# thethomasboyer/PhenDiff

Measured on AMD Instinct MI355X. Metric: img2img images/sec (50-step DDIM invert+denoise, 256x256), higher is better.
Workload: dtype bf16; 1 GPU; configs[2]: 256x256 pipeline_conditional_ddim invert->class-swap->denoise, 50+50 DDIM steps, super_small UNet (random init, seed 0), 3k_steps_clipping_rescaling, 32 images/GPU/step sharded over 1 GPU(s), no collectives; batch_per_gpu=32, global_batch=32, inference_steps=50, image_size=256, hipgraph=True, concurrent_trajectories=1

## Files before the change

### include/phendiff_hip.h

```cpp
#ifndef PHENDIFF_HIP_H_
#define PHENDIFF_HIP_H_

#include <stddef.h>
#include <stdint.h>

#ifdef __cplusplus
extern "C" {
#endif

#define PD_ABI_VERSION 8

typedef enum { PD_OK = 0, PD_ERR_ARG = -1, PD_ERR_SHAPE = -2, PD_ERR_LAUNCH = -3, PD_ERR_UNSUPPORTED = -4 } pd_status;
typedef enum { PD_F32 = 0, PD_BF16 = 1, PD_F16 = 2 } pd_dtype;
typedef enum { PD_PRED_EPSILON = 0, PD_PRED_SAMPLE = 1, PD_PRED_V = 2 } pd_pred_type;

int pd_abi_version(void);
const char* pd_last_error(void);

typedef struct {
  int rows;
  int c0;
  int tdim;
  int proj_dim;
  int flip_sin_to_cos;
// ... 44 lines not shown
  int Hout, Wout;
  int C0, C1;
  int Cout;
  int Cout_pad;
  int ksize;
  int stride;
  int pad;
  int upsample;
  int silu;
  int out_mode;
  int heads;
  const void* x0; const void* x1;
  const float* scale; const float* shift;
  const void* w_packed;
  const float* bias;
  const float* temb; int temb_stride;
  const void* residual;
  void* y;
  float* stats_out;
  const void* tail_x0; const void* tail_x1; int tail_C0, tail_C1;
  int im2col3;
  int phase;
  int phase_in;
} pd_conv_args;
int pd_conv(const pd_conv_args* a, void* stream);
int pd_conv_stat_tiles(int Hout, int Wout, int ksize, int stride);

typedef struct {
  int B, HW, groups; float eps;
  int C0, T0; const float* stats0;
  int C1, T1; const float* stats1;
  const float* gamma; const float* beta;
  float* scale; float* shift;
  float* mean; float* rstd;
  const float* temb; int temb_stride;
} pd_gn_finalize_args;
int pd_gn_finalize(const pd_gn_finalize_args* a, void* stream);

typedef struct {
  int dtype;
  int B, heads, N;
  const void* q; const void* k; const void* v;
  void* out;
  float* lse;
  const float* kmax2;
} pd_attn_args;
// ... 663 lines not shown
```

### phendiff_amd/csrc/conv_igemm.hip

```cpp
#include <type_traits>
#include <utility>
#include <stdio.h>
#include <stdlib.h>
#include "pd_common.h"
#include "pd_stage.h"
#include "pd_conv.h"

namespace pd {

constexpr int CONV_AR8 = 6;
constexpr int CONV_PRO_DEFAULT = 1;
constexpr int CONV_PRO_WPS = 3;
constexpr int CONV_PRO_START = 8;
template <int... I, typename F> __device__ __forceinline__ void pd_static_for_impl(std::integer_sequence<int, I...>, F&& f) { (f(std::integral_constant<int, I>{}), ...); }
template <int N, typename F> __device__ __forceinline__ void pd_static_for(F&& f) { pd_static_for_impl(std::make_integer_sequence<int, N>{}, f); }
constexpr int PRO_OPS = 37;
constexpr int pro_op_cost(int k) {
  if (k >= 36) return 100;
  const int stg = (k % 18) >> 1;
  return (stg == 3 || stg == 4 || stg == 6 || stg == 7) ? 87 : (stg == 0 ? 60 : (stg == 8 ? 106 : 58));
}
constexpr int pro_ops_done(int S, int NS, int PS0, int NIT) {
  if (S < PS0) return 0;
  if (S >= NS - 1) return NIT * PRO_OPS;
  long long tot = 0;
  for (int k = 0; k < PRO_OPS; ++k) tot += pro_op_cost(k);
  tot *= NIT;
  const long long target = (long long)(S - PS0 + 1) * tot / (NS - PS0);
  int done = 0;
  long long dc = 0;
  while (done < NIT * PRO_OPS && dc + pro_op_cost(done % PRO_OPS) <= target) { dc += pro_op_cost(done % PRO_OPS); ++done; }
  return done;
}
__device__ __forceinline__ unsigned pd_lin_block() { return blockIdx.x + gridDim.x * (blockIdx.y + gridDim.y * blockIdx.z); }
template <typename T, int KS, int STRIDE, int TH, int TW, bool DB, bool TAIL, int NCO = 1, bool PLAIN = false, int PRO = 0, bool STACK = false>
__global__ __launch_bounds__(256, NCO == 2 ? 2 : (PRO ? CONV_PRO_WPS : (((KS == 1 || (KS == 3 && STRIDE == 1 && TH * TW == 256)) && sizeof(T) == 2) ? 3 : 2))) void conv_kernel(const ConvP p) {
  static_assert(PRO == 0 || (!PLAIN && DB && KS == 3 && STRIDE == 1 && sizeof(T) == 2), "compile-time prologue: 16-bit 3x3 stride-1 double-buffered launches");
  static_assert(!TAIL || (DB && KS == 3 && STRIDE == 1), "fused shortcut tail: 3x3 stride-1 double-buffered variant only");
  static_assert(NCO == 1 || (NCO == 2 && DB && KS == 3 && STRIDE == 1), "two output tiles per workgroup: 3x3 stride-1 double-buffered variant only");
  static_assert(!STACK || (KS == 3 && STRIDE == 1 && TW == 8 && TH == 16 && NCO == 1 && !PLAIN && PRO == 0), "stacked 8 x 8 images: the 16 x 8 tile");
  constexpr int SG = STACK ? TH / 8 : 1;
  using E = Elem<T>;
  using Frag = typename E::Frag;
  using SR = typename Stage<T>::R;
  constexpr int TP = TH * TW;
  constexpr int NF = TP / 64;
  constexpr int RPF = 32 / TW;
  constexpr int IN_TH = STACK ? SG * 10 : (TH - 1) * STRIDE + KS;
  constexpr int IN_TW = (TW - 1) * STRIDE + KS;
  constexpr int NPIX = IN_TH * IN_TW;
  constexpr bool M16 = PLAIN && sizeof(T) == 2 && (KS == 3 || KS == 2) && STRIDE == 1 && DB && TW >= 16;
  constexpr int CHB = 32 * E::BYTES;
  constexpr int PITCH = DB ? 2 * CHB + (M16 ? 32 : 16) : CHB + 16;
  constexpr int NIT = (NPIX * 4 + 255) / 256;
  constexpr int TAPS = KS * KS;
  constexpr int KSTEPS = TAPS * 2;
  constexpr int LDS_TILE = DB ? CHB : 0;
  static_assert(RPF >= 1 && TW * RPF == 32, "TW must divide 32");

  extern __shared__ __attribute__((aligned(16))) unsigned char lds[];

  int co_t = blockIdx.y, n = blockIdx.z * SG, bx = blockIdx.x;
  if (!STACK && p.co_major) {
    const int gx = gridDim.x, gxz = gridDim.x * gridDim.z;
    const int idx = xcd_chunk_index((int)pd_lin_block(), gxz * (int)gridDim.y);
    co_t = idx / gxz;
    const int rem = idx - co_t * gxz;
    n = rem / gx; bx = rem - n * gx;
  }
  int tx, ty;
  if (p.tiles_x_shift >= 0) { tx = bx & (p.tiles_x - 1); ty = bx >> p.tiles_x_shift; }
  else { ty = bx / p.tiles_x; tx = bx - ty * p.tiles_x; }
  const int y0 = ty * TH, x0 = tx * TW;

  const int tid = threadIdx.x;
  const int lane = tid & 63;
  const int wave = __builtin_amdgcn_readfirstlane(tid >> 6);
  const int wp = wave >> 1, wc = wave & 1;
  const int r = lane & 31, h = lane >> 5;
  const int ct32 = co_t * (2 * NCO) + wc;
  const bool wave_active = (ct32 * 32) < p.Cout_pad;

  const __amdgpu_buffer_rsrc_t rs0 = __builtin_amdgcn_make_buffer_rsrc((void*)p.x0, 0, p.bytes0, 0x00020000);
  const __amdgpu_buffer_rsrc_t rs1 = __builtin_amdgcn_make_buffer_rsrc((void*)(p.x1 ? p.x1 : p.x0), 0, p.bytes1, 0x00020000);

  const __amdgpu_buffer_rsrc_t rt0 = __builtin_amdgcn_make_buffer_rsrc((void*)(TAIL ? p.t0 : p.x0), 0, TAIL ? p.tbytes0 : p.bytes0, 0x00020000);
  const __amdgpu_buffer_rsrc_t rt1 = __builtin_amdgcn_make_buffer_rsrc((void*)((TAIL && p.t1) ? p.t1 : p.x0), 0, (TAIL && p.t1) ? p.tbytes1 : p.bytes0, 0x00020000);

  const int sub = tid & 3;
  auto stage_pix = [&](int i) { return (tid + 256 * i) >> 2; };
  const int Hc = p.upsample ? p.Hin * 2 : p.Hin;
  const int Wc = p.upsample ? p.Win * 2 : p.Win;
  int spix[NIT];
  constexpr int TAIL_CENTRE = 1 << 30;
  const int ups = p.upsample ? 1 : 0;
  const int ph_mask = p.upsample >= 2 ? 1 : 0, ph_want = p.upsample == 3 ? 1 : 0;
  const int istep = p.in_step, Ws = p.Win * istep;
  const int iy_base = y0 * STRIDE - p.pad, ix_base = x0 * STRIDE - p.pad_x, n_base = n * p.Hin * istep + p.in_oy;
#pragma unroll
  for (int i = 0; i < NIT; ++i) {
    const int pix = stage_pix(i);
    const int u = pix / IN_TW, vv = pix - u * IN_TW;
    const int sj = STACK ? u / 10 : 0, su = u - sj * 10;
    const int iy = STACK ? su - 1 : iy_base + u, ix = ix_base + vv;
    const bool ok = (pix < NPIX) & ((unsigned)iy < (unsigned)Hc) & ((unsigned)ix < (unsigned)Wc) & (!STACK || n + sj < p.B)
                    & (((iy & ph_mask) == (ph_want & ph_mask)) & ((ix & ph_mask) == (ph_want & ph_mask)));
    int v = STACK ? ((n + sj) * 8 + iy) * 8 + ix : (n_base + (iy >> ups) * istep) * Ws + (ix >> ups) * istep + p.in_ox;
    if (TAIL) v |= (((unsigned)((STACK ? su : u) - KS / 2) < (unsigned)(STACK ? 8 : TH)) & ((unsigned)(vv - KS / 2) < (unsigned)TW)) ? TAIL_CENTRE : 0;
    spix[i] = ok ? v : -1;
  }
  const bool affine = PRO || (!PLAIN && p.scale != nullptr);
  const bool do_silu = PRO || (!PLAIN && p.silu != 0);
  const int cin = p.C0 + p.C1;

  SR stage[NIT];
  float sc[8], sh[8];
  bool stage_plain = false;
  auto issue_loads = [&](int chunk) {
    int src, cch;
    if (!TAIL || chunk < p.n_main) { cch = chunk * 32; src = cch < p.C0 ? 0 : 1; if (src == 1) cch -= p.C0; }
    else { cch = (chunk - p.n_main) * 32; src = cch < p.Ct0 ? 2 : 3; if (src == 3) cch -= p.Ct0; }
// ... 79 lines not shown
  };

  auto frag_row = [&](int fi, int q) { return fi * RPF + q; };
  const int li = lane & 15, lg = lane >> 4;
  constexpr int TJ_STEP = (TW >= 32 ? 16 : IN_TW) * PITCH;
  int rbase[NF];
#pragma unroll
  for (int f = 0; f < NF; ++f) {
    const int fi = wp * NF + f;
    if constexpr (M16) {
      rbase[f] = f == 0 ? ((wp * NF * RPF) * IN_TW + li) * PITCH + lg * 8 * E::BYTES : 0;
    } else {
      const int py = frag_row(fi, r / TW), px = r % TW;
      const int ly = STACK ? py + 2 * (py >> 3) : py * STRIDE;
      rbase[f] = (ly * IN_TW + px * STRIDE) * PITCH + h * 8 * E::BYTES;
    }
  }

  f32x16 acc[NCO][NF];
  f32x4 acq[NCO][NF][4];
  const int main_ksteps = (TAIL ? p.n_main : p.nchunks) * KSTEPS;
  const int all_ksteps = main_ksteps + (TAIL ? p.n_tail * 2 : 0);
  const unsigned wfrag = 512u * E::BYTES;
  const __amdgpu_buffer_rsrc_t rw = __builtin_amdgcn_make_buffer_rsrc((void*)p.w, 0, (unsigned)(p.Cout_pad / 32) * (unsigned)all_ksteps * wfrag, 0x00020000);
  const unsigned wlane = (unsigned)lane * 8u * E::BYTES;
  const unsigned wtile = (unsigned)ct32 * (unsigned)all_ksteps * wfrag;
  const unsigned wstep = 2u * (unsigned)all_ksteps * wfrag;
  auto load_w = [&](int c, int kstep) { return E::load_buf(rw, wlane, wtile + (unsigned)c * wstep + (unsigned)kstep * wfrag); };

  constexpr int AR = (KS == 3 && TW == 8 && STRIDE == 1 && sizeof(T) == 2 && TP <= 128) ? CONV_AR8 : ((KSTEPS % 3 == 0) ? 3 : 2);
  static_assert(KSTEPS % AR == 0, "the ring index is static");
  constexpr int AD = AR - 1;
  Frag aring[AR][NCO];
  static_assert(!M16 || NF % 2 == 0, "M16 walks a fragment pair per half-step");
  Frag aq[2][NCO][2];
  const unsigned wlane16 = (unsigned)(((lg >> 1) * 64 + (lg & 1) * 32 + li) * 16);
  auto load_w16 = [&](int c, int tap_index, int ti) {
    return E::load_buf(rw, wlane16 + (unsigned)ti * 256u, wtile + (unsigned)c * wstep + (unsigned)(2 * tap_index) * wfrag);
  };

  auto mma_chunk = [&](int chunk, const unsigned char* buf, unsigned char* nbuf, auto have_next_c, auto active_c) {
    constexpr int NEXT = (int)decltype(have_next_c)::value;
    constexpr bool HAVE_NEXT = NEXT != 0, NEXT_PLAIN = NEXT == 2;
    constexpr bool ACTIVE = decltype(active_c)::value;
    const int g0 = chunk * KSTEPS;
    Frag bc[NF];
    int piece = 0;
// ... 323 lines not shown
#pragma unroll
        for (int i = 0; i < 4; ++i)
          if (co + i < p.Cout) ((float*)p.y)[(((size_t)n * p.Cout + co + i) * p.Hout + oy) * p.Wout + ox] = acc[0][f][4 * g + i];
      }
    }
    return;
  }
  constexpr int EP_PITCH = 64 * E::BYTES + 16;
  constexpr int EPC = 16 / E::BYTES;
  constexpr int PPP = 64 / EPC;
  constexpr int PXI = 256 / PPP;
  constexpr int NEP = TP / PXI;
  static_assert(PXI % TW == 0 || TW % PXI == 0, "epilogue piece map");
  const int piece = tid % PPP, prow = tid / PPP;
  const int py0 = prow / TW, px0 = prow % TW;
  const int os = p.out_step, HF = p.Hout * os, WF = p.Wout * os;
  const unsigned out_bytes = (unsigned)p.B * HF * WF * p.Cout * E::BYTES;
  const __amdgpu_buffer_rsrc_t ry = __builtin_amdgcn_make_buffer_rsrc((void*)p.y, 0, p.out_mode == PD_OUT_NHWC ? out_bytes : 0u, 0x00020000);
  const __amdgpu_buffer_rsrc_t rres = __builtin_amdgcn_make_buffer_rsrc((void*)(p.residual ? p.residual : p.y), 0, p.residual ? out_bytes : 0u, 0x00020000);
  const unsigned px_bytes = (unsigned)p.Cout * E::BYTES * os, row_bytes = (unsigned)WF * p.Cout * E::BYTES * os;
  auto piece_off = [&](int it, int co) -> unsigned {
    const int dpy = (it * PXI) / TW, dpx = (it * PXI) % TW;
    const int oy = y0 + py0 + dpy, ox = x0 + px0 + dpx;
    const unsigned off = (unsigned)((n * HF + (y0 + py0) * os + p.out_oy) * WF + (x0 + px0) * os + p.out_ox) * (unsigned)(p.Cout * E::BYTES)
                         + (unsigned)co * E::BYTES + (unsigned)dpy * row_bytes + (unsigned)dpx * px_bytes;
    if constexpr (STACK) return (n + ((py0 + dpy) >> 3) < p.B && co < p.Cout) ? off : OOB_OFF;
    return (oy < p.Hout && ox < p.Wout && co < p.Cout) ? off : OOB_OFF;
  };
  if (!DB) __syncthreads();
#pragma unroll
  for (int cth = 0; cth < NCO; ++cth) {
  const int co_tile = co_t * NCO + cth;
  const int co = co_tile * 64 + piece * EPC;
  u32x4 rr[NEP];
  if (p.out_mode == PD_OUT_NHWC) {
#pragma unroll
    for (int it = 0; it < NEP; ++it) rr[it] = __builtin_amdgcn_raw_buffer_load_b128(rres, piece_off(it, co), 0, 0);
  }
  if (cth > 0) __syncthreads();
  if (wave_active) {
    if constexpr (M16) {
#pragma unroll
      for (int f = 0; f < NF; ++f)
#pragma unroll
        for (int q = 0; q < 4; ++q) {
          const int plin = (wp * NF + f) * 32 + (q & 1) * 16 + li;
          const f32x4 v = acq[cth][f][q];
// ... 67 lines not shown
    }
  }
  if (p.stats) {
    float* red = (float*)(lds + TP * EP_PITCH);
#pragma unroll
    for (int sg = 0; sg < SG; ++sg) {
      if (sg > 0) __syncthreads();
#pragma unroll
      for (int q = 0; q < 2 * EPC / 4; ++q) {
        f32x4 v4;
#pragma unroll
        for (int j = 0; j < 4; ++j) { const int e = q * 4 + j; v4[j] = e < EPC ? ssum[sg][e] : ssq[sg][e - EPC]; }
        *(f32x4*)(red + tid * (2 * EPC) + q * 4) = v4;
      }
      __syncthreads();
      if (tid < 128) {
        const int c = tid >> 1, which = tid & 1;
        const int pc = c / EPC, j = c % EPC;
        const int cog = co_tile * 64 + c;
        float tot = 0.f;
#pragma unroll 8
        for (int pr = 0; pr < PXI; ++pr) tot += red[(pr * PPP + pc) * (2 * EPC) + which * EPC + j];
        if (cog < p.Cout && n + sg < p.B) {
          const int tile = p.stat_tile_base + ty * p.tiles_x + tx;
          p.stats[(((size_t)(n + sg) * p.stat_tiles + tile) * p.Cout + cog) * 2 + which] = tot;
        }
      }
    }
  }
  }
}

template <typename T, int KS, int STRIDE, int TH, int TW, bool TAIL = false, int NCO = 1, bool PLAIN = false, int PRO = 0, bool STACK = false>
static int launch_conv(const ConvP& p, hipStream_t st) {
  constexpr int IN_TH = STACK ? (TH / 8) * 10 : (TH - 1) * STRIDE + KS, IN_TW = (TW - 1) * STRIDE + KS;
  constexpr int PITCH = 32 * Elem<T>::BYTES + 16;
  constexpr int LDS_TILE = ((IN_TH * IN_TW * PITCH + 15) / 16) * 16;
  constexpr bool DB = 2 * LDS_TILE <= 100 * 1024 && STRIDE != 2;
  constexpr bool M16 = PLAIN && sizeof(T) == 2 && (KS == 3 || KS == 2) && STRIDE == 1 && TW >= 16;
  constexpr int LDS_DB = ((IN_TH * IN_TW * (2 * 32 * Elem<T>::BYTES + (M16 ? 32 : 16)) + 15) / 16) * 16;
  constexpr int EPI_BYTES = TH * TW * (64 * Elem<T>::BYTES + 16) + 256 * 64;
  constexpr int LDS_MAIN = (DB ? LDS_DB : LDS_TILE) + (PRO ? 16 : 0);
  constexpr int LDS_BYTES = LDS_MAIN > EPI_BYTES ? LDS_MAIN : EPI_BYTES;
  static_assert(LDS_BYTES <= 160 * 1024, "tile too large");
  static_assert(NCO == 1 || DB, "NCO = 2 is a double-buffered variant");
  auto kern = conv_kernel<T, KS, STRIDE, TH, TW, DB, TAIL, NCO, PLAIN, PRO, STACK>;
  if (LDS_BYTES > 64 * 1024) {
    static LdsAttr attr;
    if (!ensure_lds(attr, kern, LDS_BYTES)) { set_error("pd_conv: cannot reserve %d bytes of LDS", LDS_BYTES); return PD_ERR_LAUNCH; }
  }
  ConvP q = p;
  q.tiles_x = (p.Wout + TW - 1) / TW;
  q.tiles_y = STACK ? 1 : (p.Hout + TH - 1) / TH;
  q.tiles_x_shift = -1;
  for (int sft = 0; sft < 16; ++sft) if ((1 << sft) == q.tiles_x) q.tiles_x_shift = sft;
  q.n_co_tiles = (p.Cout_pad + 63) / 64;
  if (q.stat_tiles == 0) q.stat_tiles = q.tiles_x * q.tiles_y;
  else { q.stat_tiles *= q.tiles_x * q.tiles_y; q.stat_tile_base *= q.tiles_x * q.tiles_y; }
  {
    const long long es = (long long)sizeof(T), cin = (long long)p.C0 + p.C1;
    const long long wbytes = (long long)p.Cout_pad * cin * KS * KS * es, abytes = (long long)p.B * p.Hin * p.Win * cin * es;
    const long long blocks = (long long)q.tiles_x * q.tiles_y * (q.n_co_tiles / NCO) * p.B;
    const int env = diag_env("PD_CONV_XCD", 0);
    q.co_major = !STACK && blocks >= 64 && blocks < (1ll << 30) && !p.im2col3 && (env == 1 || (env == 2 && wbytes > abytes));
  }
  hipLaunchKernelGGL(kern, dim3(q.tiles_x * q.tiles_y, q.n_co_tiles / NCO, STACK ? (p.B + TH / 8 - 1) / (TH / 8) : p.B), dim3(256), LDS_BYTES, st, q);
  PD_LAUNCH_CHECK();
  return PD_OK;
}

static void tile_shape(int ksize, int stride, int hout, int wout, int* th, int* tw) {
  const int tp = (ksize == 3 && stride == 1 && wout <= 8 && hout <= 8) ? 64
                 : ((ksize == 3 && stride == 2) || (ksize == 3 && stride == 1 && wout < 16 && hout <= 16)) ? 128 : 256;
  *tw = wout >= 32 ? 32 : (wout >= 16 ? 16 : 8);
  *th = tp / *tw;
}

template <typename T>
static int dispatch_conv(const ConvP& p, int ksize, int stride, hipStream_t st) {
  const int w = p.Wout;
  if (ksize == 3 && stride == 1) {
    const bool tiny = p.Hout <= 16;
    if constexpr (sizeof(T) == 2) {
      const int nco_env = diag_env("PD_CONV_NCO", 0);
      static int cus_of[16] = {0};
      int dev = 0;
      if (hipGetDevice(&dev) != hipSuccess || dev < 0 || dev >= 16) dev = 0;
      if (cus_of[dev] == 0) {
        int c = 0;
// ... 51 lines not shown
  if (ksize == 1 && stride == 1) {
    if (w >= 32) return launch_conv<T, 1, 1, 8, 32>(p, st);
    if (w >= 16) return launch_conv<T, 1, 1, 16, 16>(p, st);
    return launch_conv<T, 1, 1, 32, 8>(p, st);
  }
  set_error("pd_conv: unsupported ksize=%d stride=%d", ksize, stride);
  return PD_ERR_UNSUPPORTED;
}

}

extern "C" int pd_conv(const pd_conv_args* a, void* stream) {
  using namespace pd;
  PD_CHECK(a != nullptr, PD_ERR_ARG, "pd_conv: null args");
  PD_CHECK(a->dtype == PD_F32 || a->dtype == PD_BF16 || a->dtype == PD_F16, PD_ERR_ARG, "pd_conv: bad dtype %d", a->dtype);
  PD_CHECK(a->B > 0 && a->Hin > 0 && a->Win > 0 && a->Hout > 0 && a->Wout > 0, PD_ERR_SHAPE, "pd_conv: bad spatial shape");
  PD_CHECK(a->C0 > 0 && a->C0 % 32 == 0 && a->C1 >= 0 && a->C1 % 32 == 0, PD_ERR_SHAPE,
           "pd_conv: C0=%d C1=%d must be multiples of 32", a->C0, a->C1);
  PD_CHECK(a->Cout > 0 && a->Cout_pad >= a->Cout && a->Cout_pad % 32 == 0, PD_ERR_SHAPE, "pd_conv: bad Cout/Cout_pad");
  PD_CHECK(a->Cout % 8 == 0 || a->out_mode == PD_OUT_NCHW_F32, PD_ERR_SHAPE, "pd_conv: NHWC / head-major output needs Cout %% 8 == 0");
  PD_CHECK(a->x0 && a->w_packed && a->bias && a->y, PD_ERR_ARG, "pd_conv: null pointer");
  PD_CHECK((a->C1 == 0) == (a->x1 == nullptr), PD_ERR_ARG, "pd_conv: x1/C1 mismatch");
  PD_CHECK((a->scale == nullptr) == (a->shift == nullptr), PD_ERR_ARG, "pd_conv: scale/shift mismatch");
  PD_CHECK(a->phase >= 0 && a->phase <= 4, PD_ERR_ARG, "pd_conv: phase %d", a->phase);
  PD_CHECK(a->phase_in == 0 || (a->phase_in == 1 && a->phase), PD_ERR_ARG, "pd_conv: phase_in %d without a phase", a->phase_in);
  if (a->phase) {
    PD_CHECK(a->ksize == 2 && a->stride == 1 && !a->upsample && !a->scale && !a->silu && !a->tail_x0 && !a->im2col3 && (!a->residual || a->phase_in) &&
             a->out_mode == PD_OUT_NHWC && a->Hout == a->Hin && a->Wout == a->Win && a->C1 == 0 && !(a->phase_in && a->stats_out), PD_ERR_UNSUPPORTED,
             "pd_conv: a sub-pixel phase is a plain 2x2 convolution over one source with Hout = Hin, Wout = Win and NHWC output (residual only with phase_in, statistics only without)");
    PD_CHECK((size_t)a->B * a->Hout * a->Wout * 4 * (a->phase_in ? a->C0 : a->Cout) * (a->dtype == PD_F32 ? 4 : 2) < 0x80000000ull, PD_ERR_SHAPE,
             "pd_conv: the upsampled NHWC tensor exceeds 2 GiB (32-bit buffer offsets); split the batch");
  }
  PD_CHECK(a->ksize == 1 || a->ksize == 3 || (a->ksize == 2 && a->phase), PD_ERR_UNSUPPORTED, "pd_conv: ksize %d", a->ksize);
  PD_CHECK(a->stride == 1 || (a->stride == 2 && a->ksize == 3), PD_ERR_UNSUPPORTED, "pd_conv: stride %d", a->stride);
  PD_CHECK(!(a->upsample && a->stride != 1) && a->upsample >= 0 && a->upsample <= 3, PD_ERR_UNSUPPORTED, "pd_conv: upsample %d with stride %d", a->upsample, a->stride);
  if (!a->phase) {
    const int hc = a->upsample ? 2 * a->Hin : a->Hin, wc = a->upsample ? 2 * a->Win : a->Win;
    const int extra = (a->ksize == 3 && a->pad == 0) ? 1 : 0;
    const int ho = (hc + 2 * a->pad + extra - a->ksize) / a->stride + 1;
    const int wo = (wc + 2 * a->pad + extra - a->ksize) / a->stride + 1;
    PD_CHECK(ho == a->Hout && wo == a->Wout, PD_ERR_SHAPE, "pd_conv: Hout/Wout (%d,%d) != expected (%d,%d)", a->Hout, a->Wout, ho, wo);
  }
  if (a->out_mode == PD_OUT_QKV_HEADS)
    PD_CHECK(a->heads > 0 && a->Cout == 3 * a->heads * 8, PD_ERR_SHAPE, "pd_conv: QKV mode needs Cout == 3*heads*8");
  PD_CHECK(a->out_mode == PD_OUT_NHWC || a->residual == nullptr, PD_ERR_UNSUPPORTED, "pd_conv: residual needs NHWC output");
  if (a->im2col3) {
    PD_CHECK(a->im2col3 <= 3 && a->ksize == 1 && a->C0 == 32 && a->C1 == 0 && !a->scale && !a->upsample && a->pad == 0,
             PD_ERR_UNSUPPORTED, "pd_conv: im2col3 mode needs ksize=1, C0=32 (27 real), <= 3 source channels, no GroupNorm");
// ... 10 lines not shown
    PD_CHECK(a->tail_C0 == 0 && a->tail_C1 == 0 && a->tail_x1 == nullptr, PD_ERR_ARG, "pd_conv: tail_C without tail_x0");
  }
  const size_t esz = a->dtype == PD_F32 ? 4 : 2;
  const size_t bytes0 = (size_t)a->B * a->Hin * a->Win * a->C0 * esz * (a->phase_in ? 4 : 1), bytes1 = (size_t)a->B * a->Hin * a->Win * a->C1 * esz;
  PD_CHECK(bytes0 < 0x80000000ull && bytes1 < 0x80000000ull, PD_ERR_SHAPE,
           "pd_conv: source tensor exceeds 2 GiB (32-bit buffer offsets); split the batch");
  PD_CHECK(a->out_mode != PD_OUT_NHWC || (size_t)a->B * a->Hout * a->Wout * a->Cout * esz < 0x80000000ull, PD_ERR_SHAPE,
           "pd_conv: NHWC output exceeds 2 GiB (32-bit buffer offsets); split the batch");
  ConvP p{};
  p.B = a->B; p.Hin = a->Hin; p.Win = a->Win; p.Hout = a->Hout; p.Wout = a->Wout;
  p.C0 = a->C0; p.C1 = a->C1; p.Cout = a->Cout; p.Cout_pad = a->Cout_pad;
  p.pad = a->pad; p.upsample = a->upsample; p.silu = a->silu; p.out_mode = a->out_mode; p.heads = a->heads;
  p.n_main = (a->C0 + a->C1) / 32;
  p.n_tail = (a->tail_C0 + a->tail_C1) / 32;
  p.nchunks = p.n_main + p.n_tail;
  p.Ct0 = a->tail_C0; p.Ct1 = a->tail_C1; p.t0 = a->tail_x0; p.t1 = a->tail_x1;
  p.tbytes0 = (unsigned)((size_t)a->B * a->Hin * a->Win * a->tail_C0 * esz);
  p.tbytes1 = (unsigned)((size_t)a->B * a->Hin * a->Win * a->tail_C1 * esz);
  p.bytes0 = (unsigned)bytes0; p.bytes1 = (unsigned)(a->x1 ? bytes1 : bytes0);
  p.x0 = a->x0; p.x1 = a->x1; p.scale = a->scale; p.shift = a->shift; p.w = a->w_packed; p.bias = a->bias;
  p.temb = a->temb; p.temb_stride = a->temb_stride; p.residual = a->residual; p.y = a->y;
  p.stats = a->stats_out; p.im2col3 = a->im2col3 ? 1 : 0; p.C0r = a->im2col3;
  p.pad_x = a->pad; p.out_step = 1; p.in_step = 1;
  if (a->phase) {
    const int pa = (a->phase - 1) >> 1, pb = (a->phase - 1) & 1;
    if (a->phase_in) {
      p.pad = pa; p.pad_x = pb; p.in_step = 2; p.in_oy = pa; p.in_ox = pb;
    } else {
      p.pad = 1 - pa; p.pad_x = 1 - pb; p.out_step = 2; p.out_oy = pa; p.out_ox = pb;
      p.stat_tiles = 4; p.stat_tile_base = a->phase - 1;
    }
  }
  hipStream_t st = (hipStream_t)stream;
  if (a->dtype == PD_F32) return dispatch_conv<float>(p, a->ksize, a->stride, st);
  if (a->dtype == PD_F16) return dispatch_conv<half_t>(p, a->ksize, a->stride, st);
  return dispatch_conv<bf16_t>(p, a->ksize, a->stride, st);
}

extern "C" int pd_conv_stat_tiles(int Hout, int Wout, int ksize, int stride) {
  int th, tw;
  pd::tile_shape(ksize, stride, Hout, Wout, &th, &tw);
  return ((Hout + th - 1) / th) * ((Wout + tw - 1) / tw);
}
```

### phendiff_amd/csrc/pd_conv.h

```cpp
#pragma once
#include "pd_common.h"

namespace pd {

struct ConvP {
  int B, Hin, Win, Hout, Wout;
  int C0, C1, Cout, Cout_pad;
  int pad, upsample, silu, out_mode, heads;
  int tiles_x, tiles_y, tiles_x_shift, n_co_tiles, nchunks;
  unsigned bytes0, bytes1;
  const void* x0; const void* x1;
  const float* scale; const float* shift;
  const void* w;
  const float* bias;
  const float* temb; int temb_stride;
  const void* residual;
  void* y;
  float* stats;
  int n_main, n_tail, Ct0, Ct1;
  unsigned tbytes0, tbytes1;
  const void* t0; const void* t1;
  int im2col3;
  int C0r;
  int pad_x, out_step, out_oy, out_ox, stat_tile_base, stat_tiles;
  int in_step, in_oy, in_ox;
  int co_major;
};

}
```

### phendiff_amd/unet.py

```python
from __future__ import annotations

import ctypes as C
import json
from types import SimpleNamespace
from typing import Optional, Tuple, Union

import torch
import torch.nn as nn

from . import _lib as L
from .training import mark_requires_grad_calls
from .weight_layout import WeightSet

_DT = {"f32": (L.PD_F32, torch.float32), "bf16": (L.PD_BF16, torch.bfloat16), "fp16": (L.PD_F16, torch.float16)}

IM2COL_MAX_CHANNELS = 3
MAX_IMAGE_CHANNELS = 32


class UNet2DOutput(SimpleNamespace):
    """``diffusers.models.unet_2d.UNet2DOutput`` stand-in: ``.sample``."""


class _TimestepEmbedding(nn.Module):
# ... 332 lines not shown
    def __init__(self, fn, args, what, flops=0.0, nbytes=0.0):
        self.fn, self.args, self.what, self.flops, self.bytes = fn, args, what, float(flops), float(nbytes)
        self.ctx = False
        self.side = False


class UNetPlan:

    def __init__(self, m: CustomCondUNet2DModel, w: _PackedWeights, B, H, W, device):
        self.lib = L.lib()
        self.m, self.w = m, w
        self.B, self.H, self.W, self.device = B, H, W, device
        self.code, self.tdt = w.code, w.tdt
        c = m.config
        nlev = len(c.block_out_channels)
        if H % (1 << (nlev - 1)) or W % (1 << (nlev - 1)):
            raise ValueError(f"sample size {(H, W)} must be a multiple of {1 << (nlev - 1)}")
        self.train = bool(getattr(self, "train", False))
        self.tape = []
        self.gn_saved = {}
        self.ops = []
        self.bufs = []
        self.stats = {}
        self._kmax_arena, self._kmax_used = None, 0
        self.groups = c.norm_num_groups
        self.temb_args = None
        self._temb_ptr_fields = []
        self._in_args = None
        self._out_args = None
        self._centered = None
        self._build()

    def _esz(self):
        return 4 if self.code == L.PD_F32 else 2

    def _act(self, h, w, ch):
        t = torch.empty((self.B, h, w, ch), dtype=self.tdt, device=self.device)
        self.bufs.append(t)
        return t

    def _f32(self, *shape):
        t = torch.empty(shape, dtype=torch.float32, device=self.device)
        self.bufs.append(t)
        return t

    _sink = None

    def _emit(self, fn, args, what, flops=0.0, nbytes=0.0) -> _Op:
        op = _Op(fn, args, what, flops, nbytes)
        (self.ops if self._sink is None else self._sink).append(op)
        return op

    def _gn(self, x0, x1, gamma, beta, eps, temb_off=None):
        B, h, w, c0 = x0.shape
        c1 = x1.shape[3] if x1 is not None else 0
        C_ = c0 + c1
        st0, t0 = self.stats[id(x0)]
        st1, t1 = self.stats[id(x1)] if x1 is not None else (None, 0)
        scale, shift = self._f32(self.B, C_), self._f32(self.B, C_)
        a = L.GnFinalizeArgs(B=self.B, HW=h * w, groups=self.groups, eps=eps, C0=c0, T0=t0, stats0=st0.data_ptr(),
                             C1=c1, T1=t1, stats1=L.ptr(st1), gamma=gamma.data_ptr(), beta=beta.data_ptr(),
                             scale=scale.data_ptr(), shift=shift.data_ptr())
        if temb_off is not None:
            a.temb_stride = self.w.proj_dim
            self._temb_ptr_fields.append((a, temb_off))
        if self.train:
            mean, rstd = self._f32(self.B, self.groups), self._f32(self.B, self.groups)
            a.mean, a.rstd = mean.data_ptr(), rstd.data_ptr()
            self.gn_saved[id(scale)] = SimpleNamespace(mean=mean, rstd=rstd, gamma=gamma, beta=beta, x0=x0, x1=x1)
        self._emit(self.lib.pd_gn_finalize, a, "gn_finalize", 0.0, self.B * (t0 * c0 + t1 * c1) * 8.0)
        return scale, shift

    def _conv(self, x0, x1, wpk, bias, cout, *, ksize=3, stride=1, pad=1, upsample=0, silu=0, gn=None, temb_off=None,
              residual=None, out_mode=L.PD_OUT_NHWC, heads=0, cout_pad=None, y=None, stats=True, im2col3=0, src_ptr=None,
# ... 4 lines not shown
        extra = 1 if (ksize == 3 and pad == 0) else 0
        hout = (hc + 2 * pad + extra - ksize) // stride + 1
        wout = (wc + 2 * pad + extra - ksize) // stride + 1
        cout_pad = cout_pad or cout
        if y is None:
            if out_mode == L.PD_OUT_NHWC:
                y = self._act(hout, wout, cout)
            elif out_mode == L.PD_OUT_QKV_HEADS:
                y = torch.empty((3, B, heads, hout * wout, 8), dtype=self.tdt, device=self.device)
                self.bufs.append(y)
        st = None
        if stats and out_mode == L.PD_OUT_NHWC:
            T = self.lib.pd_conv_stat_tiles(hout, wout, ksize, stride)
            st = self._f32(B, T, cout, 2)
            self.stats[id(y)] = (st, T)
        a = L.ConvArgs(dtype=self.code, B=B, Hin=hin, Win=win, Hout=hout, Wout=wout, C0=c0, C1=c1, Cout=cout,
                       Cout_pad=cout_pad, ksize=ksize, stride=stride, pad=pad, upsample=upsample, silu=silu,
                       out_mode=out_mode, heads=heads, x0=(x0.data_ptr() if x0 is not None else src_ptr), x1=L.ptr(x1),
                       scale=L.ptr(gn[0]) if gn else None, shift=L.ptr(gn[1]) if gn else None,
                       w_packed=wpk.data_ptr(), bias=bias.data_ptr(), temb=None, temb_stride=self.w.proj_dim,
                       residual=L.ptr(residual), y=L.ptr(y), stats_out=L.ptr(st), im2col3=im2col3,
                       tail_x0=L.ptr(tail[0]) if tail else None, tail_x1=L.ptr(tail[1]) if tail else None,
                       tail_C0=tail[0].shape[3] if tail else 0,
                       tail_C1=(tail[1].shape[3] if (tail and tail[1] is not None) else 0))
        if temb_off is not None:
            self._temb_ptr_fields.append((a, temb_off))
        esz = self._esz()
        cin = c0 + c1
        flops = 2.0 * B * hout * wout * cout * cin * ksize * ksize
        tail_c = (tail[0].shape[3] + (tail[1].shape[3] if tail[1] is not None else 0)) if tail else 0
        flops += 2.0 * B * hout * wout * cout * tail_c
        nbytes = (B * hin * win * cin + B * hout * wout * cout * (2 if residual is not None else 1)) * esz \
            + cout * cin * ksize * ksize * esz + (B * hout * wout * tail_c + cout * tail_c) * esz
        if out_mode == L.PD_OUT_NCHW_F32:
            nbytes += B * hout * wout * cout * (4 - esz)
        self._emit(self.lib.pd_conv, a, what or f"conv{ksize}x{ksize}", flops, nbytes)
        return y, a

    @property
    def SUBPIXEL_UP(self):
        return __import__("os").environ.get("PD_SUBPIXEL_UP", "1") != "0"


    def _subpixel_up_ok(self, x):
        B, h, w, ch = x.shape
        esz = self._esz()
        return (self.SUBPIXEL_UP and (not getattr(self, "train", False) or getattr(self, "subpixel_in_training", False)) and w >= 16 and ch % 32 == 0
                and B * 4 * h * w * ch * esz < (1 << 31))

    def _upconv_subpixel(self, x, s):
        B, h, w, ch = x.shape
        y = self._act(2 * h, 2 * w, ch)
        T = self.lib.pd_conv_stat_tiles(h, w, 2, 1)
        st = self._f32(B, 4 * T, ch, 2)
        self.stats[id(y)] = (st, 4 * T)
        esz = self._esz()
        for ph in range(4):
            a = L.ConvArgs(dtype=self.code, B=B, Hin=h, Win=w, Hout=h, Wout=w, C0=ch, C1=0, Cout=ch, Cout_pad=ch, ksize=2, stride=1, pad=0,
                           upsample=0, silu=0, out_mode=L.PD_OUT_NHWC, heads=0, x0=x.data_ptr(), x1=None, scale=None, shift=None,
                           w_packed=s.w4[ph].data_ptr(), bias=s.b.data_ptr(), temb=None, temb_stride=self.w.proj_dim, residual=None,
                           y=y.data_ptr(), stats_out=st.data_ptr(), im2col3=0, tail_x0=None, tail_x1=None, tail_C0=0, tail_C1=0, phase=1 + ph)
            self._emit(self.lib.pd_conv, a, "conv3x3", 2.0 * B * 4 * h * w * ch * ch * 9 / 4.0,
                       (B * h * w * ch + B * 4 * h * w * ch) * esz / 4.0 + ch * ch * 4 * esz)
        return y

    PREAPPLY_MIN_COUT = int(__import__("os").environ.get("PD_PREAPPLY_MIN_COUT", 320))

    def _gn_apply(self, x0, x1, gn, silu, what="gn_apply"):
        B, h, w, c0 = x0.shape
        c1 = x1.shape[3] if x1 is not None else 0
        y = self._act(h, w, c0 + c1)
        a = L.GnApplyArgs(dtype=self.code, B=B, HW=h * w, C0=c0, C1=c1, silu=silu, x0=x0.data_ptr(), x1=L.ptr(x1),
                          scale=gn[0].data_ptr(), shift=gn[1].data_ptr(), y=y.data_ptr())
        self._emit(self.lib.pd_gn_apply, a, what, 0.0, 2.0 * y.numel() * self._esz())
        return y

    def _linear(self, x, wpk, bias, cout, residual=None, y=None, gn=None, stats=False, what="linear", glu=False):
        B, h, w, K = x.shape
        if y is None:
            y = self._act(h, w, cout // 2 if glu else cout)
        M, esz = B * h * w, self._esz()
        st = None
        if stats:
            T = (h * w) // 128
            st = self._f32(B, T, cout, 2)
            self.stats[id(y)] = (st, T)
        a = L.LinearArgs(dtype=self.code, M=M, K=K, N=cout, N_pad=((cout + 31) // 32) * 32, x=x.data_ptr(), x_stride=K,
                         w_packed=wpk.data_ptr(), bias=bias.data_ptr(), residual=L.ptr(residual), y=y.data_ptr(),
                         scale=L.ptr(gn[0]) if gn else None, shift=L.ptr(gn[1]) if gn else None, rows_per_sample=h * w, qkv_heads=0,
                         stats_out=L.ptr(st), glu=int(glu))
        self._emit(self.lib.pd_linear, a, what, 2.0 * M * K * cout,
                   (M * K + M * (cout // 2 if glu else cout) * (2 if residual is not None else 1) + K * cout) * esz)
        return y

    @staticmethod
    def _linear_ok(x):
        return (x.shape[1] * x.shape[2]) % 128 == 0 and x.shape[3] % 64 == 0

    def _resnet(self, name, x0, x1=None):
        e = self.w.resnets[name]
        pre = e.cout >= self.PREAPPLY_MIN_COUT
        z1 = z2 = None
        ss = getattr(e, "scale_shift", False)
        t1 = None if ss else e.temb_off
        gn1 = self._gn(x0, x1, e.g1, e.be1, e.eps)
        if pre:
            z1 = self._gn_apply(x0, x1, gn1, 1)
            h1, _ = self._conv(z1, None, e.w1, e.b1, e.cout, temb_off=t1)
        else:
            h1, _ = self._conv(x0, x1, e.w1, e.b1, e.cout, silu=1, gn=gn1, temb_off=t1)
        gn2 = self._gn(h1, None, e.g2, e.be2, e.eps, temb_off=e.temb_off if ss else None)
        if pre:
            z2 = self._gn_apply(h1, None, gn2, 1)
        src, kw = (z2, dict()) if pre else (h1, dict(silu=1, gn=gn2))
        if e.fused_shortcut:
# ... 21 lines not shown
        e = self.w.attns[name]
        B, h, w, ch = x.shape
        if ch != e.heads * 8:
            return self._attn_nhwc(name, x)
        gn = self._gn(x, None, e.g, e.be, e.eps)
        if (h * w) % 128 == 0 and ch % 64 == 0:
            qkv = torch.empty((3, B, e.heads, h * w, 8), dtype=self.tdt, device=self.device)
            self.bufs.append(qkv)
            M = B * h * w
            kmax2 = self._kmax_slot(B * e.heads) if self.code != L.PD_F32 else None
            a = L.LinearArgs(dtype=self.code, M=M, K=ch, N=3 * ch, N_pad=3 * ch, x=x.data_ptr(), x_stride=ch, w_packed=e.wqkv.data_ptr(),
                             bias=e.bqkv.data_ptr(), residual=None, y=qkv.data_ptr(), scale=gn[0].data_ptr(), shift=gn[1].data_ptr(),
                             rows_per_sample=h * w, qkv_heads=e.heads, kmax2_out=kmax2)
            need = int(self.lib.pd_linear_fold_workspace(C.byref(a))) if __import__("os").environ.get("PD_LIN_FOLD", "0") != "0" else 0
            if need > 0:
                ws = getattr(self, "_fold_ws", None)
                if ws is None or ws.numel() < need:
                    ws = torch.empty(need, dtype=torch.uint8, device=self.device)
                    self._fold_ws = ws
                    self.bufs.append(ws)
                a.fold_ws, a.fold_ws_bytes = ws.data_ptr(), need
            esz_ = self._esz()
            self._emit(self.lib.pd_linear, a, "conv1x1", 2.0 * M * ch * 3 * ch, (M * ch * 4 + 3 * ch * ch) * esz_)
        else:
            kmax2 = None
            qkv, _ = self._conv(x, None, e.wqkv, e.bqkv, 3 * ch, ksize=1, pad=0, gn=gn, out_mode=L.PD_OUT_QKV_HEADS,
                                heads=e.heads)
        o = self._act(h, w, ch)
        lse = self._f32(B, e.heads, h * w) if self.train else None
        a = L.AttnArgs(dtype=self.code, B=B, heads=e.heads, N=h * w, q=qkv[0].data_ptr(), k=qkv[1].data_ptr(),
                       v=qkv[2].data_ptr(), out=o.data_ptr(), lse=L.ptr(lse), kmax2=kmax2)
        esz = self._esz()
        N = h * w
        self._emit(self.lib.pd_attn_d8, a, "attn_d8", 4.0 * B * e.heads * N * N * 8, 4.0 * B * N * ch * esz)
        if self._linear_ok(o):
            out = self._linear(o, e.wo, e.bo, ch, residual=x, stats=True, what="conv1x1")
        else:
            out, _ = self._conv(o, None, e.wo, e.bo, ch, ksize=1, pad=0, residual=x)
        self.tape.append(SimpleNamespace(kind="attn", name=name, x=x, qkv=qkv, o=o, out=out, lse=lse, gn=gn, e=e))
        return out

    def _attn_nhwc(self, name, x):
        e = self.w.attns[name]
        B, h, w, ch = x.shape
        N, esz = h * w, self._esz()
        d = ch // e.heads
        if d not in (16, 32, 64, 128, 256, 512):
            raise NotImplementedError(f"attention head_dim {d}: implemented are 8, 16, 32, 64 and one wide head of 128 / 256 / 512 channels")
        gn = self._gn(x, None, e.g, e.be, e.eps)
        qkv, _ = self._conv(x, None, e.wqkv, e.bqkv, 3 * ch, ksize=1, pad=0, gn=gn, stats=False)
        o = self._act(h, w, ch)
        p = qkv.data_ptr()
        lse = self._f32(B, e.heads, N) if self.train else None
        if d == 64:
            a = L.AttnD64Args(dtype=self.code, B=B, heads=e.heads, Nq=N, Nkv=N, q=p, q_stride=3 * ch, k=p + ch * esz,
                              v=p + 2 * ch * esz, kv_stride=3 * ch, out=o.data_ptr(), out_stride=ch, lse=L.ptr(lse))
            fn, what = self.lib.pd_attn_d64, "attn_d64"
        elif d in (16, 32):
            a = L.AttnHdArgs(dtype=self.code, B=B, heads=e.heads, D=d, Nq=N, Nkv=N, scale=float(d) ** -0.5, q=p, q_stride=3 * ch,
                             k=p + ch * esz, v=p + 2 * ch * esz, kv_stride=3 * ch, out=o.data_ptr(), out_stride=ch, lse=L.ptr(lse))
            fn, what = self.lib.pd_attn_hd, "attn_hd"
        else:
            a = L.AttnWideArgs(dtype=self.code, B=B, heads=e.heads, D=d, Nq=N, Nkv=N, scale=float(d) ** -0.5, q=p, q_stride=3 * ch,
                               k=p + ch * esz, v=p + 2 * ch * esz, kv_stride=3 * ch, out=o.data_ptr(), out_stride=ch, lse=L.ptr(lse))
            fn, what = self.lib.pd_attn_wide, "attn_wide"
        self._emit(fn, a, what, 4.0 * B * N * N * ch, 4.0 * B * N * ch * esz)
        if self._linear_ok(o):
            out = self._linear(o, e.wo, e.bo, ch, residual=x, stats=True, what="conv1x1")
        else:
            out, _ = self._conv(o, None, e.wo, e.bo, ch, ksize=1, pad=0, residual=x)
        self.tape.append(SimpleNamespace(kind="attn_nhwc", name=name, x=x, qkv=qkv, o=o, out=out, lse=lse, gn=gn, e=e, d=d))
        return out

    def _build(self):
        m, w, c = self.m, self.w, self.m.config
        boc = c.block_out_channels
        B, H, W = self.B, self.H, self.W
        self.temb_args = L.TembArgs(rows=B, c0=boc[0], tdim=m.time_embed_dim, proj_dim=w.proj_dim,
                                    flip_sin_to_cos=int(c.flip_sin_to_cos), freq_shift=float(c.freq_shift),
                                    num_classes=(c.num_class_embeds or 0), w1=w.w1T.data_ptr(), b1=w.b1.data_ptr(),
                                    w2=w.w2T.data_ptr(), b2=w.b2.data_ptr(), class_table=L.ptr(w.class_table),
                                    wp=w.wpT.data_ptr(), bp=w.bp.data_ptr())
        self._in_field = "x0"
        centered = None
        if c.center_input_sample:
            centered = self._f32(B, c.in_channels, H, W)
            self._centered = centered
            self._center_const = (torch.ones_like(centered), torch.full((B,), 2.0, device=self.device), torch.full((B,), -1.0, device=self.device))
            ones, two, neg = self._center_const
# ... 163 lines not shown
```

Baseline: 15.98 images/s.

## Alternate conv grid traversal direction and fuse four upsample phases into one launch

Adds a grid_order flag that makes a conv launch walk its workgroups in reverse when the previous producer of its input walked forward. The later conv then first reads the tiles written last, which are more likely still in L2/MALL cache. Separately, the four 2x2 phase convolutions of the upsampler are merged into one launch (phase 5) that picks each phase's weights and offsets from the block index. This removes three launches per upsample but adds some per-block index math and early-exit blocks.

```diff
diff --git a/include/phendiff_hip.h b/include/phendiff_hip.h
--- a/include/phendiff_hip.h
+++ b/include/phendiff_hip.h
@@ -90,6 +90,8 @@
   int im2col3;
   int phase;
   int phase_in;
+  int grid_order;
+  const void *w_phase2, *w_phase3, *w_phase4;
 } pd_conv_args;
 int pd_conv(const pd_conv_args* a, void* stream);
 int pd_conv_stat_tiles(int Hout, int Wout, int ksize, int stride);
diff --git a/phendiff_amd/csrc/conv_igemm.hip b/phendiff_amd/csrc/conv_igemm.hip
--- a/phendiff_amd/csrc/conv_igemm.hip
+++ b/phendiff_amd/csrc/conv_igemm.hip
@@ -32,7 +32,6 @@
   while (done < NIT * PRO_OPS && dc + pro_op_cost(done % PRO_OPS) <= target) { dc += pro_op_cost(done % PRO_OPS); ++done; }
   return done;
 }
-__device__ __forceinline__ unsigned pd_lin_block() { return blockIdx.x + gridDim.x * (blockIdx.y + gridDim.y * blockIdx.z); }
 template <typename T, int KS, int STRIDE, int TH, int TW, bool DB, bool TAIL, int NCO = 1, bool PLAIN = false, int PRO = 0, bool STACK = false>
 __global__ __launch_bounds__(256, NCO == 2 ? 2 : (PRO ? CONV_PRO_WPS : (((KS == 1 || (KS == 3 && STRIDE == 1 && TH * TW == 256)) && sizeof(T) == 2) ? 3 : 2))) void conv_kernel(const ConvP p) {
   static_assert(PRO == 0 || (!PLAIN && DB && KS == 3 && STRIDE == 1 && sizeof(T) == 2), "compile-time prologue: 16-bit 3x3 stride-1 double-buffered launches");
@@ -60,13 +59,29 @@
 
   extern __shared__ __attribute__((aligned(16))) unsigned char lds[];
 
-  int co_t = blockIdx.y, n = blockIdx.z * SG, bx = blockIdx.x;
+  const unsigned gbx = p.grid_order ? gridDim.x - 1 - blockIdx.x : blockIdx.x;
+  const unsigned gby = p.grid_order ? gridDim.y - 1 - blockIdx.y : blockIdx.y;
+  const unsigned gbz = p.grid_order ? gridDim.z - 1 - blockIdx.z : blockIdx.z;
+  int co_t = gby, n = gbz * SG, bx = gbx;
   if (!STACK && p.co_major) {
     const int gx = gridDim.x, gxz = gridDim.x * gridDim.z;
-    const int idx = xcd_chunk_index((int)pd_lin_block(), gxz * (int)gridDim.y);
+    const int idx = xcd_chunk_index((int)(gbx + gridDim.x * (gby + gridDim.y * gbz)), gxz * (int)gridDim.y);
     co_t = idx / gxz;
     const int rem = idx - co_t * gxz;
     n = rem / gx; bx = rem - n * gx;
+  }
+  int pad = p.pad, pad_x = p.pad_x, out_oy = p.out_oy, out_ox = p.out_ox, stat_tile_base = p.stat_tile_base;
+  const void* wsrc = p.w;
+  if constexpr (KS == 2) {
+    if (p.phase4) {
+      const int ph = (bx >> 3) & 3, tiles = p.tiles_x * p.tiles_y;
+      bx = ((bx >> 5) << 3) | (bx & 7);
+      if (bx >= tiles) return;
+      const int pa = ph >> 1, pb = ph & 1;
+      pad = 1 - pa; pad_x = 1 - pb; out_oy = pa; out_ox = pb;
+      stat_tile_base = ph * tiles;
+      wsrc = ph == 0 ? p.w : p.wph[ph - 1];
+    }
   }
   int tx, ty;
   if (p.tiles_x_shift >= 0) { tx = bx & (p.tiles_x - 1); ty = bx >> p.tiles_x_shift; }
@@ -96,7 +111,7 @@
   const int ups = p.upsample ? 1 : 0;
   const int ph_mask = p.upsample >= 2 ? 1 : 0, ph_want = p.upsample == 3 ? 1 : 0;
   const int istep = p.in_step, Ws = p.Win * istep;
-  const int iy_base = y0 * STRIDE - p.pad, ix_base = x0 * STRIDE - p.pad_x, n_base = n * p.Hin * istep + p.in_oy;
+  const int iy_base = y0 * STRIDE - pad, ix_base = x0 * STRIDE - pad_x, n_base = n * p.Hin * istep + p.in_oy;
 #pragma unroll
   for (int i = 0; i < NIT; ++i) {
     const int pix = stage_pix(i);
@@ -222,7 +237,7 @@
   const int main_ksteps = (TAIL ? p.n_main : p.nchunks) * KSTEPS;
   const int all_ksteps = main_ksteps + (TAIL ? p.n_tail * 2 : 0);
   const unsigned wfrag = 512u * E::BYTES;
-  const __amdgpu_buffer_rsrc_t rw = __builtin_amdgcn_make_buffer_rsrc((void*)p.w, 0, (unsigned)(p.Cout_pad / 32) * (unsigned)all_ksteps * wfrag, 0x00020000);
+  const __amdgpu_buffer_rsrc_t rw = __builtin_amdgcn_make_buffer_rsrc((void*)wsrc, 0, (unsigned)(p.Cout_pad / 32) * (unsigned)all_ksteps * wfrag, 0x00020000);
   const unsigned wlane = (unsigned)lane * 8u * E::BYTES;
   const unsigned wtile = (unsigned)ct32 * (unsigned)all_ksteps * wfrag;
   const unsigned wstep = 2u * (unsigned)all_ksteps * wfrag;
@@ -592,7 +607,7 @@
   auto piece_off = [&](int it, int co) -> unsigned {
     const int dpy = (it * PXI) / TW, dpx = (it * PXI) % TW;
     const int oy = y0 + py0 + dpy, ox = x0 + px0 + dpx;
-    const unsigned off = (unsigned)((n * HF + (y0 + py0) * os + p.out_oy) * WF + (x0 + px0) * os + p.out_ox) * (unsigned)(p.Cout * E::BYTES)
+    const unsigned off = (unsigned)((n * HF + (y0 + py0) * os + out_oy) * WF + (x0 + px0) * os + out_ox) * (unsigned)(p.Cout * E::BYTES)
                          + (unsigned)co * E::BYTES + (unsigned)dpy * row_bytes + (unsigned)dpx * px_bytes;
     if constexpr (STACK) return (n + ((py0 + dpy) >> 3) < p.B && co < p.Cout) ? off : OOB_OFF;
     return (oy < p.Hout && ox < p.Wout && co < p.Cout) ? off : OOB_OFF;
@@ -706,7 +721,7 @@
 #pragma unroll 8
         for (int pr = 0; pr < PXI; ++pr) tot += red[(pr * PPP + pc) * (2 * EPC) + which * EPC + j];
         if (cog < p.Cout && n + sg < p.B) {
-          const int tile = p.stat_tile_base + ty * p.tiles_x + tx;
+          const int tile = stat_tile_base + ty * p.tiles_x + tx;
           p.stats[(((size_t)(n + sg) * p.stat_tiles + tile) * p.Cout + cog) * 2 + which] = tot;
         }
       }
@@ -746,9 +761,10 @@
     const long long wbytes = (long long)p.Cout_pad * cin * KS * KS * es, abytes = (long long)p.B * p.Hin * p.Win * cin * es;
     const long long blocks = (long long)q.tiles_x * q.tiles_y * (q.n_co_tiles / NCO) * p.B;
     const int env = diag_env("PD_CONV_XCD", 0);
-    q.co_major = !STACK && blocks >= 64 && blocks < (1ll << 30) && !p.im2col3 && (env == 1 || (env == 2 && wbytes > abytes));
-  }
-  hipLaunchKernelGGL(kern, dim3(q.tiles_x * q.tiles_y, q.n_co_tiles / NCO, STACK ? (p.B + TH / 8 - 1) / (TH / 8) : p.B), dim3(256), LDS_BYTES, st, q);
+    q.co_major = !STACK && blocks >= 64 && blocks < (1ll << 30) && !p.im2col3 && !p.phase4 && (env == 1 || (env == 2 && wbytes > abytes));
+  }
+  const int grid_x = (KS == 2 && p.phase4) ? ((q.tiles_x * q.tiles_y + 7) / 8) * 32 : q.tiles_x * q.tiles_y;
+  hipLaunchKernelGGL(kern, dim3(grid_x, q.n_co_tiles / NCO, STACK ? (p.B + TH / 8 - 1) / (TH / 8) : p.B), dim3(256), LDS_BYTES, st, q);
   PD_LAUNCH_CHECK();
   return PD_OK;
 }
@@ -846,8 +862,13 @@
   PD_CHECK(a->x0 && a->w_packed && a->bias && a->y, PD_ERR_ARG, "pd_conv: null pointer");
   PD_CHECK((a->C1 == 0) == (a->x1 == nullptr), PD_ERR_ARG, "pd_conv: x1/C1 mismatch");
   PD_CHECK((a->scale == nullptr) == (a->shift == nullptr), PD_ERR_ARG, "pd_conv: scale/shift mismatch");
-  PD_CHECK(a->phase >= 0 && a->phase <= 4, PD_ERR_ARG, "pd_conv: phase %d", a->phase);
-  PD_CHECK(a->phase_in == 0 || (a->phase_in == 1 && a->phase), PD_ERR_ARG, "pd_conv: phase_in %d without a phase", a->phase_in);
+  PD_CHECK(a->phase >= 0 && a->phase <= 5, PD_ERR_ARG, "pd_conv: phase %d", a->phase);
+  PD_CHECK(a->phase_in == 0 || (a->phase_in == 1 && a->phase >= 1 && a->phase <= 4), PD_ERR_ARG, "pd_conv: phase_in %d without a phase 1..4 (phase %d)", a->phase_in, a->phase);
+  PD_CHECK(a->grid_order == 0 || a->grid_order == 1, PD_ERR_ARG, "pd_conv: grid_order %d", a->grid_order);
+  if (a->phase == 5)
+    PD_CHECK(a->w_phase2 && a->w_phase3 && a->w_phase4, PD_ERR_ARG, "pd_conv: phase 5 (all four phases) needs w_phase2, w_phase3 and w_phase4");
+  else
+    PD_CHECK(!a->w_phase2 && !a->w_phase3 && !a->w_phase4, PD_ERR_ARG, "pd_conv: w_phase2..4 without phase 5");
   if (a->phase) {
     PD_CHECK(a->ksize == 2 && a->stride == 1 && !a->upsample && !a->scale && !a->silu && !a->tail_x0 && !a->im2col3 && (!a->residual || a->phase_in) &&
              a->out_mode == PD_OUT_NHWC && a->Hout == a->Hin && a->Wout == a->Win && a->C1 == 0 && !(a->phase_in && a->stats_out), PD_ERR_UNSUPPORTED,
@@ -904,7 +925,11 @@
   p.temb = a->temb; p.temb_stride = a->temb_stride; p.residual = a->residual; p.y = a->y;
   p.stats = a->stats_out; p.im2col3 = a->im2col3 ? 1 : 0; p.C0r = a->im2col3;
   p.pad_x = a->pad; p.out_step = 1; p.in_step = 1;
-  if (a->phase) {
+  p.grid_order = a->grid_order;
+  if (a->phase == 5) {
+    p.phase4 = 1; p.out_step = 2; p.stat_tiles = 4; p.stat_tile_base = 0;
+    p.wph[0] = a->w_phase2; p.wph[1] = a->w_phase3; p.wph[2] = a->w_phase4;
+  } else if (a->phase) {
     const int pa = (a->phase - 1) >> 1, pb = (a->phase - 1) & 1;
     if (a->phase_in) {
       p.pad = pa; p.pad_x = pb; p.in_step = 2; p.in_oy = pa; p.in_ox = pb;
diff --git a/phendiff_amd/csrc/pd_conv.h b/phendiff_amd/csrc/pd_conv.h
--- a/phendiff_amd/csrc/pd_conv.h
+++ b/phendiff_amd/csrc/pd_conv.h
@@ -25,6 +25,9 @@
   int pad_x, out_step, out_oy, out_ox, stat_tile_base, stat_tiles;
   int in_step, in_oy, in_ox;
   int co_major;
+  int grid_order;
+  int phase4;
+  const void* wph[3];
 };
 
 }
diff --git a/phendiff_amd/unet.py b/phendiff_amd/unet.py
--- a/phendiff_amd/unet.py
+++ b/phendiff_amd/unet.py
@@ -378,6 +378,7 @@
         self.ops = []
         self.bufs = []
         self.stats = {}
+        self._dir = {}
         self._kmax_arena, self._kmax_used = None, 0
         self.groups = c.norm_num_groups
         self.temb_args = None
@@ -406,6 +407,30 @@
         op = _Op(fn, args, what, flops, nbytes)
         (self.ops if self._sink is None else self._sink).append(op)
         return op
+
+    _dir = None
+
+    @property
+    def GRID_ORDER(self):
+        return __import__("os").environ.get("PD_CONV_GRID_ORDER", "1") != "0"
+
+    @property
+    def UP_ONE_LAUNCH(self):
+        return __import__("os").environ.get("PD_UP_ONE_LAUNCH", "1") != "0"
+
+    def _flip(self, src, dst):
+        if self._sink is not None or not self.GRID_ORDER:
+            return 0
+        if self._dir is None:
+            self._dir = {}
+        d = 1 - self._dir.get(id(src), 1)
+        if dst is not None:
+            self._dir[id(dst)] = d
+        return d
+
+    def _same_dir(self, src, dst):
+        if self._dir is not None and id(src) in self._dir:
+            self._dir[id(dst)] = self._dir[id(src)]
 
     def _gn(self, x0, x1, gamma, beta, eps, temb_off=None):
         B, h, w, c0 = x0.shape
@@ -456,7 +481,7 @@
                        residual=L.ptr(residual), y=L.ptr(y), stats_out=L.ptr(st), im2col3=im2col3,
                        tail_x0=L.ptr(tail[0]) if tail else None, tail_x1=L.ptr(tail[1]) if tail else None,
                        tail_C0=tail[0].shape[3] if tail else 0,
-                       tail_C1=(tail[1].shape[3] if (tail and tail[1] is not None) else 0))
+                       tail_C1=(tail[1].shape[3] if (tail and tail[1] is not None) else 0), grid_order=self._flip(x0, y))
         if temb_off is not None:
             self._temb_ptr_fields.append((a, temb_off))
         esz = self._esz()
@@ -489,11 +514,20 @@
         st = self._f32(B, 4 * T, ch, 2)
         self.stats[id(y)] = (st, 4 * T)
         esz = self._esz()
+        order = self._flip(x, y)
+        if self.UP_ONE_LAUNCH and not getattr(self, "train", False) and self._sink is None:
+            a = L.ConvArgs(dtype=self.code, B=B, Hin=h, Win=w, Hout=h, Wout=w, C0=ch, C1=0, Cout=ch, Cout_pad=ch, ksize=2, stride=1, pad=0,
+                           upsample=0, silu=0, out_mode=L.PD_OUT_NHWC, heads=0, x0=x.data_ptr(), x1=None, scale=None, shift=None,
+                           w_packed=s.w4[0].data_ptr(), w_phase2=s.w4[1].data_ptr(), w_phase3=s.w4[2].data_ptr(), w_phase4=s.w4[3].data_ptr(),
+                           bias=s.b.data_ptr(), temb=None, temb_stride=self.w.proj_dim, residual=None, y=y.data_ptr(), stats_out=st.data_ptr(),
+                           im2col3=0, tail_x0=None, tail_x1=None, tail_C0=0, tail_C1=0, phase=5, grid_order=order)
+            self._emit(self.lib.pd_conv, a, "conv3x3", 2.0 * B * 4 * h * w * ch * ch * 9, (B * h * w * ch + B * 4 * h * w * ch) * esz + 4 * ch * ch * 4 * esz)
+            return y
         for ph in range(4):
             a = L.ConvArgs(dtype=self.code, B=B, Hin=h, Win=w, Hout=h, Wout=w, C0=ch, C1=0, Cout=ch, Cout_pad=ch, ksize=2, stride=1, pad=0,
                            upsample=0, silu=0, out_mode=L.PD_OUT_NHWC, heads=0, x0=x.data_ptr(), x1=None, scale=None, shift=None,
                            w_packed=s.w4[ph].data_ptr(), bias=s.b.data_ptr(), temb=None, temb_stride=self.w.proj_dim, residual=None,
-                           y=y.data_ptr(), stats_out=st.data_ptr(), im2col3=0, tail_x0=None, tail_x1=None, tail_C0=0, tail_C1=0, phase=1 + ph)
+                           y=y.data_ptr(), stats_out=st.data_ptr(), im2col3=0, tail_x0=None, tail_x1=None, tail_C0=0, tail_C1=0, phase=1 + ph, grid_order=order)
             self._emit(self.lib.pd_conv, a, "conv3x3", 2.0 * B * 4 * h * w * ch * ch * 9 / 4.0,
                        (B * h * w * ch + B * 4 * h * w * ch) * esz / 4.0 + ch * ch * 4 * esz)
         return y
@@ -507,6 +541,7 @@
         a = L.GnApplyArgs(dtype=self.code, B=B, HW=h * w, C0=c0, C1=c1, silu=silu, x0=x0.data_ptr(), x1=L.ptr(x1),
                           scale=gn[0].data_ptr(), shift=gn[1].data_ptr(), y=y.data_ptr())
         self._emit(self.lib.pd_gn_apply, a, what, 0.0, 2.0 * y.numel() * self._esz())
+        self._same_dir(x0, y)
         return y
 
     def _linear(self, x, wpk, bias, cout, residual=None, y=None, gn=None, stats=False, what="linear", glu=False):
@@ -525,6 +560,7 @@
                          stats_out=L.ptr(st), glu=int(glu))
         self._emit(self.lib.pd_linear, a, what, 2.0 * M * K * cout,
                    (M * K + M * (cout // 2 if glu else cout) * (2 if residual is not None else 1) + K * cout) * esz)
+        self._same_dir(x, y)
         return y
 
     @staticmethod
@@ -592,6 +628,7 @@
                 a.fold_ws, a.fold_ws_bytes = ws.data_ptr(), need
             esz_ = self._esz()
             self._emit(self.lib.pd_linear, a, "conv1x1", 2.0 * M * ch * 3 * ch, (M * ch * 4 + 3 * ch * ch) * esz_)
+            self._same_dir(x, qkv)
         else:
             kmax2 = None
             qkv, _ = self._conv(x, None, e.wqkv, e.bqkv, 3 * ch, ksize=1, pad=0, gn=gn, out_mode=L.PD_OUT_QKV_HEADS,
@@ -603,6 +640,7 @@
         esz = self._esz()
         N = h * w
         self._emit(self.lib.pd_attn_d8, a, "attn_d8", 4.0 * B * e.heads * N * N * 8, 4.0 * B * N * ch * esz)
+        self._same_dir(qkv, o)
         if self._linear_ok(o):
             out = self._linear(o, e.wo, e.bo, ch, residual=x, stats=True, what="conv1x1")
         else:
@@ -635,6 +673,7 @@
                                k=p + ch * esz, v=p + 2 * ch * esz, kv_stride=3 * ch, out=o.data_ptr(), out_stride=ch, lse=L.ptr(lse))
             fn, what = self.lib.pd_attn_wide, "attn_wide"
         self._emit(fn, a, what, 4.0 * B * N * N * ch, 4.0 * B * N * ch * esz)
+        self._same_dir(qkv, o)
         if self._linear_ok(o):
             out = self._linear(o, e.wo, e.bo, ch, residual=x, stats=True, what="conv1x1")
         else:
```

Result: no change. 16.11 images/s, median of 6 (+0.8%).
